# Tiago27Cruz/OctreeRayTracer

Hardware: AMD Instinct MI355X
Metric: Mrays/sec at 3840x2160, 100k spheres, depth 8; 1/2/4/8-GPU scaling (higher is better)
Workload: dtype f32; 1 GPU; c3: 3840x2160 camera rays (spp=1, bounces=1), 100000 spheres, octree depth 8, maxSpheresPerNode 0; width=3840, height=2160, spheres=100000, octree_depth=8, max_spheres_per_node=0, num_samples=1, max_bounces=1, nodes=10953681, indices=5472144, layout=compact, partition=full frame, frames_in_flight=2, rays=traced rays (octree traversals), all bounces and ranks

## Files before the change

octreeraytracer_amd/csrc/host_emulation.inc:

```

namespace {

struct HostScene {
    enum Check {
        kValidate = 1,
        kNoOctree = 2,
        kValidateTree = 4,
        kOrdered = 8,
    };
    ort::KScene S;
    int mode = 2;
    ort::CompactLayout cl;
    std::vector<float> fplanes, fplanes_b;
    std::vector<uint8_t> lut;
    std::vector<uint4> leaf16;
    std::vector<uint2> cam_node;
    const uint8_t* rank_lut = nullptr;
    std::string error;
    HostScene() { std::memset(&S, 0, sizeof(S)); }
    HostScene(const HostScene&) = delete;
    HostScene& operator=(const HostScene&) = delete;

    int build(const float* cr, const float* ma, const float* fr, int32_t n_spheres, const float* node_min, const float* node_max,
              const int32_t* co, const int32_t* oo, const int32_t* cnt, int32_t n_nodes, const int32_t* idx, int64_t n_indices,
// ... 12 lines not shown
            fr2_.resize((size_t)n_spheres * 2);
            for (int32_t i = 0; i < n_spheres; ++i) {
                fr2_[2 * (size_t)i] = fr[4 * (size_t)i];
                fr2_[2 * (size_t)i + 1] = fr[4 * (size_t)i + 1];
            }
            S.sph_ma = (const float4*)ma;
            S.sph_fr = (const float2*)fr2_.data();
        }
        S.n_spheres = n_spheres;
        S.n_nodes = n_nodes;
        lut.resize(kRankLutBytes);
        for (size_t i = 0; i < lut.size(); ++i) lut[i] = ort::rank_lut_entry((uint32_t)i >> 8, (uint32_t)i & 255u);
        if (!tree) return ORT_OK;
        if (layout == ORT_LAYOUT_COMPACT) {
            if (!ort::buildCompactLayout(in, ORT_COMPACT_MAX_DEPTH, cl, error)) return ORT_ERR_UNSUPPORTED;
            if ((checks & kOrdered) && !cl.ordered) return error = "unordered tree", ORT_ERR_UNSUPPORTED;
            mode = 0;
            S.node = (const uint2*)cl.node.data();
            S.kid = (const uint2*)cl.kid.data();
            S.tail_base = (uint32_t)in.n_indices;
            S.leaf_sph = (const float4*)cl.leaf_sph.data();
            S.leaf_idx = cl.leaf_idx.data();
            S.planes = cl.planes.data();
            S.depth = cl.depth;
            if (ort::Masks64::kLeafInline && cl.depth <= 8) {
                fill_leaf16((const uint2*)cl.node.data(), (int64_t)(cl.node.size() / 2), (const uint4*)cl.leaf_sph.data(),
                            (int64_t)(cl.leaf_sph.size() / 4), leaf16);
                S.leaf16 = leaf16.data();
                S.leaf16_bytes = (uint32_t)(16 * leaf16.size());
                if (ort::Masks64::kLeafDedup) {
                    fill_cam_node((const uint2*)cl.node.data(), leaf16, cam_node);
                    S.cam_node = cam_node.data();
                    S.cam_bytes = (uint32_t)(8 * cam_node.size());
                }
            }
            fplanes.resize(ort::fast_plane_floats(cl.depth));
            ort::fill_fast_planes(cl.planes.data(), fplanes.data(), cl.depth);
            fplanes_b.resize(ort::fast_plane_floats(cl.depth, true));
            ort::fill_fast_planes(cl.planes.data(), fplanes_b.data(), cl.depth, true);
            if (cl.ordered) rank_lut = lut.data();
            return ORT_OK;
        }
        mode = 1;
        a_.resize(4 * (size_t)n_nodes);
        b_.resize(4 * (size_t)n_nodes);
        for (int32_t i = 0; i < n_nodes; ++i) {
            for (int k = 0; k < 3; ++k) {
                a_[4 * (size_t)i + k] = node_min[3 * (size_t)i + k];
                b_[4 * (size_t)i + k] = node_max[3 * (size_t)i + k];
            }
            std::memcpy(&a_[4 * (size_t)i + 3], &co[i], 4);
            std::memcpy(&b_[4 * (size_t)i + 3], &oo[i], 4);
        }
        S.nodeA = (const float4*)a_.data();
        S.nodeB = (const float4*)b_.data();
        S.count = cnt;
        S.indices = idx;
        return ORT_OK;
    }

    static void fill_leaf16(const uint2* node, int64_t n, const uint4* leaf_sph, int64_t n_ent, std::vector<uint4>& out) {
        out.resize((size_t)n);
        for (int64_t i = 0; i < n; ++i) {
            const uint2 rec = node[i];
            uint4 sp = make_uint4(0u, 0u, 0u, ort::kLeaf16ListTag);
            if (rec.y == 1u && (int64_t)rec.x < n_ent) sp = leaf_sph[rec.x];
            out[(size_t)i] = ort::leaf16_record(rec, sp);
        }
    }

    static void fill_cam_node(const uint2* node, const std::vector<uint4>& leaf16, std::vector<uint2>& out) {
        const int64_t n = (int64_t)leaf16.size();
        out.resize((size_t)n);
        for (int64_t i = 0; i < n; ++i) {
            const uint2 rec = node[i];
            const uint32_t ab = ort::cam_has_masks(rec, n) ? ort::leaf_repeat_masks(&leaf16[rec.x], rec.y & 0xffu) : 0u;
            out[(size_t)i] = ort::cam_record(rec, ab);
        }
    }

private:
    std::vector<float> zeros_, fr2_, a_, b_;
};

}

extern "C" {

int ort_debug_trace_rays(const float* cr, int32_t n_spheres, const float* node_min, const float* node_max,
                         const int32_t* co, const int32_t* oo, const int32_t* cnt, int32_t n_nodes, const int32_t* idx,
                         int64_t n_indices, const float* rays, int32_t n_rays, int32_t bounce, int32_t* out) {
    try {
        HostScene hs;
        if (int rc = hs.build(cr, nullptr, nullptr, n_spheres, node_min, node_max, co, oo, cnt, n_nodes, idx, n_indices,
                              ORT_LAYOUT_COMPACT, 1, HostScene::kValidate | HostScene::kOrdered))
            return fail(nullptr, rc, hs.error);
        const ort::KScene& S = hs.S;
        const std::vector<float>&fplanes = hs.fplanes, &fplanes_b = hs.fplanes_b;
        const std::vector<uint8_t>& lut = hs.lut;
        ort::LocalFrames lf;
        for (int32_t i = 0; i < n_rays; ++i) {
            ort::Ray r;
            r.o = ort::mk(rays[6 * (size_t)i], rays[6 * (size_t)i + 1], rays[6 * (size_t)i + 2]);
            r.d = ort::mk(rays[6 * (size_t)i + 3], rays[6 * (size_t)i + 4], rays[6 * (size_t)i + 5]);
            ort::Counters cc;
            for (int k = 0; k < 6; ++k) cc.v[k] = 0;
            float tf = 0.0f, tx = 0.0f;
            int ef = -1, ex = -1;
            ort::V3 inv = ort::mk(1.0f / r.d.x, 1.0f / r.d.y, 1.0f / r.d.z);
            const bool fast = ort::fast_prepare(S, r, inv);
            if (fast) {
                if (!bounce) ort::traverse_fast<false>(S, fplanes.data(), lut.data(), r, inv, 0.001f, ORT_MAXFLOAT, ef, tf, lf, cc);
                else if (S.depth <= 8)
                    ort::traverse_fast_t<false, ort::Masks64Plain>(S, fplanes.data(), lut.data(), r, inv, 0.001f, ORT_MAXFLOAT,
                                                                 ef, tf, lf, cc);
                else
                    ort::traverse_fast_t<false, ort::Masks96Lean>(S, fplanes_b.data(), lut.data(), r, inv, 0.001f,
                                                                ORT_MAXFLOAT, ef, tf, lf, cc);
            }
            ort::traverse_compact<false>(S, fplanes.data(), r, 0.001f, ORT_MAXFLOAT, ex, tx, lf, cc);
            int32_t* o = out + 5 * (size_t)i;
            o[0] = fast ? 1 : 0;
            o[1] = ef;
            o[2] = (int32_t)ort::f2u(tf);
            o[3] = ex;
            o[4] = (int32_t)ort::f2u(tx);
        }
        return ORT_OK;
    } catch (const std::exception& ex) {
        return fail(nullptr, ORT_ERR_INTERNAL, ex.what());
    }
}

int ort_debug_split_rays(const float* cr, int32_t n_spheres, const float* node_min, const float* node_max,
                         const int32_t* co, const int32_t* oo, const int32_t* cnt, int32_t n_nodes, const int32_t* idx,
                         int64_t n_indices, const float* rays, int32_t n_rays, int32_t level, int32_t lanes, int32_t* out) {
    try {
        if (lanes < 1 || level < 1) return fail(nullptr, ORT_ERR_INVALID_ARG, "ort_debug_split_rays: lanes, level >= 1");
        HostScene hs;
        if (int rc = hs.build(cr, nullptr, nullptr, n_spheres, node_min, node_max, co, oo, cnt, n_nodes, idx, n_indices,
                              ORT_LAYOUT_COMPACT, 1, HostScene::kValidate | HostScene::kOrdered))
            return fail(nullptr, rc, hs.error);
        const ort::KScene& S = hs.S;
        const std::vector<float>& fplanes = hs.fplanes;
        const std::vector<uint8_t>& lut = hs.lut;
        ort::LocalFrames lf;
        for (int32_t i = 0; i < n_rays; ++i) {
            ort::Ray r;
            r.o = ort::mk(rays[6 * (size_t)i], rays[6 * (size_t)i + 1], rays[6 * (size_t)i + 2]);
            r.d = ort::mk(rays[6 * (size_t)i + 3], rays[6 * (size_t)i + 4], rays[6 * (size_t)i + 5]);
            const ort::V3 inv = ort::mk(1.0f / r.d.x, 1.0f / r.d.y, 1.0f / r.d.z);
            int32_t* o = out + 4 * (size_t)i;
            o[0] = -1;
            o[1] = 0;
            o[2] = 0x7fffffff;
            o[3] = 0;
            if (!ort::fast_path_ok(r, inv, 0.001f, ORT_MAXFLOAT)) continue;
            int best = 0x7fffffff, be = -1, top = 0, owns = 0;
            float bt = 0.0f;
            for (int j = 0; j < lanes; ++j) {
                int pos = 0x7fffffff, e = -1, st = 0, own = 0;
                float t = 0.0f;
                if (S.depth > 8)
                    ort::traverse_split<ort::Masks96Split>(S, fplanes.data(), lut.data(), r, inv, level, lanes, j, pos, e, t, lf, st, own);
                else
                    ort::traverse_split<ort::Masks64Split>(S, fplanes.data(), lut.data(), r, inv, level, lanes, j, pos, e, t, lf, st, own);
// ... 435 lines not shown
    try {
        if (!name || !bytes) return fail(nullptr, ORT_ERR_INVALID_ARG, "ort_debug_layout: null argument");
        HostScene hs;
        if (int rc = hs.build(cr, nullptr, nullptr, n_spheres, node_min, node_max, co, oo, cnt, n_nodes, idx, n_indices,
                              ORT_LAYOUT_COMPACT, 1, HostScene::kValidate))
            return fail(nullptr, rc, hs.error);
        const std::string what = name;
        const int32_t depth = hs.cl.depth, ordered = hs.cl.ordered ? 1 : 0;
        const void* src = nullptr;
        size_t n = 0;
        if (what == "node") src = hs.cl.node.data(), n = 4 * hs.cl.node.size();
        else if (what == "kid") src = hs.cl.kid.data(), n = 4 * hs.cl.kid.size();
        else if (what == "leaf_sph") src = hs.cl.leaf_sph.data(), n = 4 * hs.cl.leaf_sph.size();
        else if (what == "leaf_idx") src = hs.cl.leaf_idx.data(), n = 4 * hs.cl.leaf_idx.size();
        else if (what == "planes") src = hs.cl.planes.data(), n = 4 * hs.cl.planes.size();
        else if (what == "leaf16") src = hs.leaf16.data(), n = 16 * hs.leaf16.size();
        else if (what == "cam_node") src = hs.cam_node.data(), n = 8 * hs.cam_node.size();
        else if (what == "depth") src = &depth, n = 4;
        else if (what == "ordered") src = &ordered, n = 4;
        else return fail(nullptr, ORT_ERR_INVALID_ARG, "ort_debug_layout: unknown array " + what);
        *bytes = (int64_t)n;
        if (!out || n == 0) return ORT_OK;
        if (cap_bytes < (int64_t)n) return fail(nullptr, ORT_ERR_INVALID_ARG, "ort_debug_layout: out too small");
        std::memcpy(out, src, n);
        return ORT_OK;
    } catch (const std::exception& ex) {
        return fail(nullptr, ORT_ERR_INTERNAL, ex.what());
    }
}

int ort_debug_ctx_array(ort_ctx* ctx, const char* name, void* out, int64_t cap_bytes, int64_t* bytes) {
    if (!ctx || !name || !bytes) return fail(ctx, ORT_ERR_INVALID_ARG, "ort_debug_ctx_array: null argument");
    if (!ctx->scene.has_scene) return fail(ctx, ORT_ERR_NO_SCENE, "ort_debug_ctx_array: no scene");
    const std::string what = name;
    const Scene& sc = ctx->scene;
    const int32_t scalars[3] = {sc.depth, sc.ordered ? 1 : 0, sc.layout};
    const char* const scalar_names[3] = {"depth", "ordered", "layout"};
    for (int k = 0; k < 3; ++k)
        if (what == scalar_names[k]) {
            *bytes = 4;
            if (!out) return ORT_OK;
            if (cap_bytes < 4) return fail(ctx, ORT_ERR_INVALID_ARG, "ort_debug_ctx_array: out too small");
            std::memcpy(out, &scalars[k], 4);
            return ORT_OK;
        }
    const DevBuf* b = nullptr;
    if (what == "node") b = &sc.node;
    else if (what == "kid") b = &sc.kid;
    else if (what == "leaf_sph") b = &sc.leaf_sph;
    else if (what == "leaf_idx") b = &sc.leaf_idx;
    else if (what == "planes") b = &sc.planes;
    else if (what == "nk") b = &sc.nk;
    else if (what == "leaf16") b = &sc.leaf16;
    else if (what == "cam_node") b = &sc.cam_node;
    else if (what == "lds_img") b = &sc.lds_img;
    else if (what == "lds_rev") b = &sc.lds_rev;
    else return fail(ctx, ORT_ERR_INVALID_ARG, "ort_debug_ctx_array: unknown array " + what);
    *bytes = b->p ? (int64_t)b->bytes : 0;
    if (!out || *bytes == 0) return ORT_OK;
    if (cap_bytes < *bytes) return fail(ctx, ORT_ERR_INVALID_ARG, "ort_debug_ctx_array: out too small");
    HIPCHK(ctx, hipSetDevice(ctx->device));
    HIPCHK(ctx, hipStreamSynchronize(ctx->stream));
    HIPCHK(ctx, hipMemcpy(out, b->p, b->bytes, hipMemcpyDeviceToHost));
    return ORT_OK;
}

int ort_debug_leaf_forms(uint64_t* out4, int32_t reset) {
    for (int i = 0; i < 4; ++i) {
        if (out4) out4[i] = ort::g_leaf_forms[i];
        if (reset) ort::g_leaf_forms[i] = 0;
    }
    return ORT_OK;
}

int ort_debug_leaf_dedup(uint64_t* out3, int32_t reset) {
    for (int i = 0; i < 2; ++i) {
        if (out3) out3[i] = ort::g_leaf_dedup[i];
        if (reset) ort::g_leaf_dedup[i] = 0;
    }
    if (out3) out3[2] = (uint64_t)ort::Masks64::kLeafDedup;
    return ORT_OK;
}

int ort_debug_pop_coverage(uint64_t* hb_pops, uint64_t* sign_masks, int32_t reset) {
    for (int i = 0; i < 64; ++i)
        if (hb_pops) hb_pops[i] = ort::g_pop_cover[i];
    for (int i = 0; i < 8; ++i)
        if (sign_masks) sign_masks[i] = ort::g_pop_cover[64 + i];
    if (reset)
        for (int i = 0; i < 72; ++i) ort::g_pop_cover[i] = 0;
    return ORT_OK;
}

}
```

octreeraytracer_amd/csrc/ort_internal.h:

```cpp
#pragma once
#include <cstdint>
#include <string>

#include "../../include/ort.h"

namespace ort {
void set_thread_error(const std::string& msg);
const char* thread_error();
}

extern "C" {
int ort_debug_emulate_render(const float* sphere_center_radius, const float* sphere_mat_albedo,
                             const float* sphere_fuzz_ri, int32_t n_spheres, const float* node_min,
                             const float* node_max, const int32_t* children_offset,
                             const int32_t* objects_offset, const int32_t* object_count, int32_t n_nodes,
                             const int32_t* object_indices, int64_t n_indices, int32_t layout,
                             const ort_params* params, const ort_tile* tile, float* rgb_out, uint64_t* counts);
int ort_debug_emulate_render_prefix(const float* sphere_center_radius, const float* sphere_mat_albedo,
                                    const float* sphere_fuzz_ri, int32_t n_spheres, const float* node_min,
                                    const float* node_max, const int32_t* children_offset,
                                    const int32_t* objects_offset, const int32_t* object_count, int32_t n_nodes,
                                    const int32_t* object_indices, int64_t n_indices, int32_t layout,
                                    const ort_params* params, const ort_tile* tile, int32_t samples_done,
                                    float* rgb_out, uint64_t* counts);
// ... 13 lines not shown
                         const float* node_max, const int32_t* children_offset, const int32_t* objects_offset,
                         const int32_t* object_count, int32_t n_nodes, const int32_t* object_indices, int64_t n_indices,
                         const float* rays, int32_t n_rays, int32_t bounce, int32_t* out);
int ort_debug_query_rays(const float* sphere_center_radius, int32_t n_spheres, const float* node_min,
                         const float* node_max, const int32_t* children_offset, const int32_t* objects_offset,
                         const int32_t* object_count, int32_t n_nodes, const int32_t* object_indices, int64_t n_indices,
                         int32_t layout, int32_t use_octree, const float* rays, int64_t n_rays, ort_ray_hit* hits,
                         float* normals);
int ort_debug_query_rays_ex(const float* sphere_center_radius, int32_t n_spheres, const float* node_min,
                            const float* node_max, const int32_t* children_offset, const int32_t* objects_offset,
                            const int32_t* object_count, int32_t n_nodes, const int32_t* object_indices, int64_t n_indices,
                            int32_t layout, int32_t use_octree, const float* rays, int64_t n_rays, int32_t mode,
                            const float* t_range, ort_ray_hit* hits, float* normals);
int ort_debug_camera_query(const float* sphere_center_radius, int32_t n_spheres, const float* node_min,
                           const float* node_max, const int32_t* children_offset, const int32_t* objects_offset,
                           const int32_t* object_count, int32_t n_nodes, const int32_t* object_indices, int64_t n_indices,
                           int32_t layout, const ort_params* params, const ort_tile* tile, int32_t which, float* rays,
                           ort_ray_hit* hits, float* normals);
int ort_debug_radiance_rays(const float* sphere_center_radius, const float* sphere_mat_albedo,
                            const float* sphere_fuzz_ri, int32_t n_spheres, const float* node_min,
                            const float* node_max, const int32_t* children_offset, const int32_t* objects_offset,
                            const int32_t* object_count, int32_t n_nodes, const int32_t* object_indices,
                            int64_t n_indices, int32_t layout, int32_t use_octree, const float* rays,
                            const float* states, int64_t n_rays, int32_t max_depth, int32_t paths, int32_t flags,
                            float* radiance, float* states_out);
int ort_debug_denoise(const ort_denoise_desc* d, const ort_output* output);
int ort_debug_denoise_ex(const ort_denoise_desc_ex* d, const ort_output* output);
int ort_debug_history_update(const ort_params* prev_params, int32_t prev_x0, int32_t prev_y0, const float* prev_a,
                             const float* prev_b, const ort_history_frame* f, float* next_a, float* next_b);
int ort_debug_history_update_ex(const ort_params* prev_params, int32_t prev_x0, int32_t prev_y0, const float* prev_a,
                                const float* prev_b, const ort_history_frame_ex* f, const float* now, const float* snap,
                                int32_t n_spheres, float* next_a, float* next_b);
int ort_debug_history_state(int64_t* st, int32_t op, int32_t n_spheres, int32_t* reads_snapshot);
int ort_debug_gamma(const float* rgb, int64_t n_pixels, float* out);
int ort_debug_emulate_moments(const float* sphere_center_radius, const float* sphere_mat_albedo,
                              const float* sphere_fuzz_ri, int32_t n_spheres, const float* node_min,
                              const float* node_max, const int32_t* children_offset,
                              const int32_t* objects_offset, const int32_t* object_count, int32_t n_nodes,
                              const int32_t* object_indices, int64_t n_indices, int32_t layout,
                              const ort_params* params, const ort_tile* tile, int32_t samples_done,
                              float* mean, float* variance);
int ort_debug_emulate_adaptive(const float* sphere_center_radius, const float* sphere_mat_albedo,
                               const float* sphere_fuzz_ri, int32_t n_spheres, const float* node_min,
                               const float* node_max, const int32_t* children_offset,
                               const int32_t* objects_offset, const int32_t* object_count, int32_t n_nodes,
                               const int32_t* object_indices, int64_t n_indices, int32_t layout,
                               const ort_params* params, const ort_tile* tile, const ort_accum_adaptive* passes,
                               int32_t n_passes, int32_t* counts, float* mean, float* variance);
int ort_debug_adaptive_decision(int32_t k, int32_t n_total, const ort_accum_adaptive* criterion, const float* col, float m2);
int ort_debug_wave_stats(const float* sphere_center_radius, const float* sphere_mat_albedo,
                         const float* sphere_fuzz_ri, int32_t n_spheres, const float* node_min,
                         const float* node_max, const int32_t* children_offset, const int32_t* objects_offset,
                         const int32_t* object_count, int32_t n_nodes, const int32_t* object_indices,
                         int64_t n_indices, const ort_params* params, int32_t block_step, double* stats,
                         int32_t n_stats);
int ort_debug_bounce_walks(const float* sphere_center_radius, const float* sphere_mat_albedo,
                           const float* sphere_fuzz_ri, int32_t n_spheres, const float* node_min, const float* node_max,
                           const int32_t* children_offset, const int32_t* objects_offset, const int32_t* object_count,
                           int32_t n_nodes, const int32_t* object_indices, int64_t n_indices, const ort_params* params,
                           const ort_tile* tile, int32_t bounce, float* rays, int32_t* walks, int64_t cap,
                           int64_t* n_out);
int64_t ort_debug_walk_steps(const float* sphere_center_radius, const float* sphere_mat_albedo,
                             const float* sphere_fuzz_ri, int32_t n_spheres, const float* node_min,
                             const float* node_max, const int32_t* children_offset, const int32_t* objects_offset,
                             const int32_t* object_count, int32_t n_nodes, const int32_t* object_indices,
                             int64_t n_indices, const ort_params* params, int32_t block_step, int32_t* lens,
                             int64_t n_lens, uint16_t* steps, int64_t cap);
int ort_debug_lds_image(int32_t depth, const float* planes, uint32_t* image, int64_t cap_words, int32_t* layout);
int ort_debug_pop_coverage(uint64_t* hb_pops, uint64_t* sign_masks, int32_t reset);
int ort_debug_leaf16(const float* sphere_center_radius, int32_t n_spheres, const float* node_min, const float* node_max,
                     const int32_t* children_offset, const int32_t* objects_offset, const int32_t* object_count,
                     int32_t n_nodes, const int32_t* object_indices, int64_t n_indices, uint32_t* node,
                     uint32_t* leaf_sph, uint32_t* leaf16, int64_t* sizes);
int ort_debug_ctx_leaf16(ort_ctx* ctx, uint32_t* out, int64_t cap, int64_t* n);
int ort_debug_lds_image_rev(int32_t depth, const float* planes, int32_t rev_tables, uint32_t* image, int64_t cap_words,
                            int32_t* layout);
int ort_debug_layout(const float* sphere_center_radius, int32_t n_spheres, const float* node_min, const float* node_max,
                     const int32_t* children_offset, const int32_t* objects_offset, const int32_t* object_count,
                     int32_t n_nodes, const int32_t* object_indices, int64_t n_indices, const char* name, void* out,
                     int64_t cap_bytes, int64_t* bytes);
int ort_debug_ctx_array(ort_ctx* ctx, const char* name, void* out, int64_t cap_bytes, int64_t* bytes);
int ort_debug_leaf_forms(uint64_t* out4, int32_t reset);
int ort_debug_leaf_dedup(uint64_t* out3, int32_t reset);
int64_t ort_debug_walk_steps_ex(const float* sphere_center_radius, const float* sphere_mat_albedo, const float* sphere_fuzz_ri,
                                int32_t n_spheres, const float* node_min, const float* node_max, const int32_t* children_offset,
                                const int32_t* objects_offset, const int32_t* object_count, int32_t n_nodes,
                                const int32_t* object_indices, int64_t n_indices, const ort_params* p, int32_t block_step,
                                int32_t production, int32_t* lens, int64_t n_lens, uint16_t* steps, int64_t cap);
}
```

octreeraytracer_amd/csrc/render_fast_state.inc:

```
namespace ort {
struct Masks64 {
    static constexpr bool kLdsScene = false;
    static constexpr bool kInlineLeaves = true;
    static constexpr bool kRevPlanes = true;
    static constexpr bool kPreMid = true;
    static constexpr bool kKidSkip = false;
    static constexpr bool kPopTable = true;
    static constexpr bool kLeafInline = true;
    static constexpr bool kLeafDedup = true;
    uint64_t m;
    ORT_FN void clear() { m = 0; }
    ORT_FN bool empty() const { return m == 0; }
    ORT_FN void put(int L, uint32_t rev) { m |= (uint64_t)rev << (8 * L); }
    ORT_FN int pop() {
        const int hb = 63 - __builtin_clzll(m);
        m ^= (uint64_t)1 << hb;
        return hb;
    }
    ORT_FN int peek() const { return 63 - __builtin_clzll(m); }
    ORT_FN void drop(uint32_t lo, uint32_t hi) { m ^= ((uint64_t)hi << 32) | lo; }
    ORT_FN bool take(int hb) {
        const uint64_t b = (uint64_t)1 << hb;
        const bool t = (m & b) != 0;
        m &= ~b;
        return t;
    }
    ORT_FN void uniform() {
#if defined(__HIP_DEVICE_COMPILE__)
        m = ((uint64_t)(uint32_t)__builtin_amdgcn_readfirstlane((int)(uint32_t)(m >> 32)) << 32) |
            (uint32_t)__builtin_amdgcn_readfirstlane((int)(uint32_t)m);
#endif
    }
};
struct Masks96 {
    static constexpr bool kLdsScene = false;
    static constexpr bool kInlineLeaves = false;
    static constexpr bool kLeafInline = false;
    static constexpr bool kLeafDedup = false;
    static constexpr bool kPreMid = false;
    static constexpr bool kRevPlanes = false;
    static constexpr bool kPopTable = false;
    static constexpr bool kKidSkip = true;
    static constexpr int kSplit = 2;
    uint64_t lo;
    uint32_t hi;
    ORT_FN void clear() { lo = 0; hi = 0; }
    ORT_FN bool empty() const { return (lo | hi) == 0; }
    ORT_FN void put(int L, uint32_t rev) {
        if (L >= kSplit) lo |= (uint64_t)rev << (8 * (L - kSplit));
        else hi |= rev << (8 * L);
    }
    ORT_FN int pop() {
        if (lo) {
            const int hb = 63 - __builtin_clzll(lo);
            lo ^= (uint64_t)1 << hb;
            return 8 * kSplit + hb;
        }
        const int hb = 31 - __builtin_clz(hi);
        hi ^= 1u << hb;
        return hb;
    }
    ORT_FN bool take(int hb) {
        if (hb >= 8 * kSplit) {
            const uint64_t b = (uint64_t)1 << (hb - 8 * kSplit);
            const bool t = (lo & b) != 0;
            lo &= ~b;
            return t;
        }
        const uint32_t b = 1u << hb;
        const bool t = (hi & b) != 0;
        hi &= ~b;
        return t;
    }    ORT_FN void uniform() {
#if defined(__HIP_DEVICE_COMPILE__)
        lo = ((uint64_t)(uint32_t)__builtin_amdgcn_readfirstlane((int)(uint32_t)(lo >> 32)) << 32) |
             (uint32_t)__builtin_amdgcn_readfirstlane((int)(uint32_t)lo);
        hi = (uint32_t)__builtin_amdgcn_readfirstlane((int)hi);
#endif
    }
};

template <class Masks>
struct FastStateT {
    static_assert(!Masks::kPreMid || (Masks::kRevPlanes && Masks::kInlineLeaves), "mid planes in the pop: never a level-D leaf");
    static_assert(!Masks::kPopTable || (Masks::kRevPlanes && Masks::kInlineLeaves), "the pop table has no level-D entries");
    static_assert(!Masks::kLeafInline || (Masks::kInlineLeaves && !Masks::kKidSkip), "leaf16 records: inline leaf children, no skip");
    static_assert(!Masks::kLeafDedup || Masks::kLeafInline, "repeat masks: the leaf16 records");
    V3 d;
    float ya;
    float oA, oB, oC, iA, iB, iC;
    const float* pl0;
    uint32_t aA, aB, aC;
    uint32_t h4;
#if defined(__HIP_DEVICE_COMPILE__)
    ORT_FN float plane(uint32_t a) const { return *(const __attribute__((address_space(3))) float*)(size_t)a; }
    static ORT_FN uint32_t table_base(const float* planes) {
        return (uint32_t)(size_t)(const __attribute__((address_space(3))) float*)planes;
    }
    ORT_FN uint4 entry(uint32_t a) const { return *(const __attribute__((address_space(3))) uint4*)(size_t)a; }
#else
    ORT_FN float plane(uint32_t off) const { return *(const float*)((const char*)pl0 + off); }
    ORT_FN uint4 entry(uint32_t off) const {
        uint4 e;
        __builtin_memcpy(&e, (const char*)pl0 + off, 16);
        return e;
    }
    static ORT_FN uint32_t table_base(const float*) { return 0u; }
#endif
    const float* pA;
    const float* pB;
    const float* pC;
    int sA, sB, sC;
    float tNA, tFA, tNB, tFB, tNC, tFC;
    float tMA, tMB, tMC;
    uint32_t cP;
    uint32_t otab;
    int node, depth;
    uint2 kd;
    uint2 rec;
    float closest;
    int hitEntry;
    uint32_t kc_id;
    float kc_e;
    Masks masks;
    ORT_FN bool hit() const { return hitEntry >= 0; }
    ORT_FN float pl(const float* p, int s, int idx) const { return *at(p, s, idx); }
    const float* nA;
    const float* nB;
    const float* nC;
    ORT_FN const float* at(const float* p, int s, int idx) const {
        return (const float*)((const char*)p + imul24(s, idx));
    }
    ORT_FN float plA(int idx) const { return pl(pA, sA, idx); }
    ORT_FN float plB(int idx) const { return pl(pB, sB, idx); }
    ORT_FN float plC(int idx) const { return pl(pC, sC, idx); }
    ORT_FN int cA() const { return (int)(cP & 1023u); }
    ORT_FN int cB() const { return (int)((cP >> 10) & 1023u); }
    ORT_FN int cC() const { return (int)(cP >> 20); }
    ORT_FN Ray ray() const {
        const bool swap = (otab >> 1) & 1u;
        Ray r;
        r.o = mk(swap ? oB : oA, swap ? oA : oB, oC);
        r.d = d;
        return r;
    }
};
using FastState = FastStateT<Masks96>;
struct Masks96Lean : Masks96 {
    static constexpr bool kRevPlanes = true;
};
struct Masks64Plain : Masks64 {
    static constexpr bool kInlineLeaves = false;
    static constexpr bool kLeafInline = false;
    static constexpr bool kLeafDedup = false;
    static constexpr bool kPopTable = false;
    static constexpr bool kPreMid = false;
    static constexpr bool kKidSkip = true;
};
struct Masks64PlainLds : Masks64Plain {
    static constexpr bool kLdsScene = true;
};

struct Masks64Split : Masks64Plain {
    static constexpr bool kKidSkip = false;
};
struct Masks96Split : Masks96 {
    static constexpr bool kKidSkip = false;
};
}
```

octreeraytracer_amd/csrc/render_fast_walk.inc:

```
namespace ort {
#if defined(__HIP_DEVICE_COMPILE__)
ORT_FN uint4 lds_u4(uint32_t a) { return *(const __attribute__((address_space(3))) uint4*)(size_t)a; }
#endif
template <bool CAM = false, class Masks>
ORT_FN void fetch_rec(const KScene& S, int i, bool kid, FastStateT<Masks>& st) {
    if constexpr (CAM) {
        static_assert(!Masks::kKidSkip && !Masks::kLdsScene, "cam_node: the depth <= 8 camera walk, no kid entries");
        st.rec = fetch_cam(S, i);
        return;
    }
#if defined(__HIP_DEVICE_COMPILE__)
    if constexpr (Masks::kLdsScene) {
        const uint4 v = lds_u4(S.lds_nk + 16u * (uint32_t)i);
        st.rec = make_uint2(v.x, v.y);
        st.kd = make_uint2(v.z, v.w);
        return;
    }
#endif
    if (Masks::kKidSkip && kid && S.nk) {
        const uint4 v = fetch_nk(S, i);
        st.rec = make_uint2(v.x, v.y);
        st.kd = make_uint2(v.z, v.w);
        return;
    }
    st.rec = fetch_node(S, i);
    if (kid) st.kd = fetch_kid(S, i);
}

template <int CAM = -1, class Masks>
ORT_FN bool fast_begin(const KScene& S, const float* planes, const uint8_t* rank_lut, const Ray& r, V3 inv, float t_min,
                       float t_max, FastStateT<Masks>& st) {
    const int D = S.depth;
    const int top = 1 << D;
    const uint32_t nx = f2u(inv.x) >> 31, ny = f2u(inv.y) >> 31, nz = f2u(inv.z) >> 31;
    const uint32_t m = (nz << 2) | (nx << 1) | ny;
    const bool swap = nx != 0;
    const uint32_t gA = swap ? ny : nx, gB = swap ? nx : ny, gC = nz;
    st.d = r.d;
    st.ya = 1.0f / dot(r.d, r.d);
    st.oA = swap ? r.o.y : r.o.x;
    st.oB = swap ? r.o.x : r.o.y;
    st.oC = r.o.z;
    st.iA = swap ? inv.y : inv.x;
    st.iB = swap ? inv.x : inv.y;
    st.iC = inv.z;
    st.otab = (swap ? 0x75643120u : 0x76543210u) ^ (m * 0x11111111u);
    if (Masks::kRevPlanes) {
        st.pl0 = planes;
        const uint32_t b0 = FastStateT<Masks>::table_base(planes);
        const uint32_t T = (uint32_t)fast_rev_T(D), S3 = 3u * T;
        st.aA = b0 + 4u * ((swap ? S3 : 0u) + (gA ? T : 0u));
        st.aB = b0 + 4u * ((swap ? 0u : S3) + (gB ? T : 0u));
        st.aC = b0 + 4u * (2u * S3 + (gC ? T : 0u));
        st.h4 = 2u * (uint32_t)top;
        const uint32_t t4 = 4u * (uint32_t)top;
        st.tNA = st.iA * (st.plane(st.aA) - st.oA);
        st.tFA = st.iA * (st.plane(st.aA + t4) - st.oA);
        st.tNB = st.iB * (st.plane(st.aB) - st.oB);
        st.tFB = st.iB * (st.plane(st.aB + t4) - st.oB);
        st.tNC = st.iC * (st.plane(st.aC) - st.oC);
        st.tFC = st.iC * (st.plane(st.aC + t4) - st.oC);
        if (Masks::kPreMid) {
            const uint32_t hm = st.h4 & ~3u;
            st.tMA = st.iA * (st.plane(st.aA + hm) - st.oA);
            st.tMB = st.iB * (st.plane(st.aB + hm) - st.oB);
            st.tMC = st.iC * (st.plane(st.aC + hm) - st.oC);
        }
    } else {
        const int S1 = fast_axis_floats(D);
        st.pA = planes + (swap ? S1 : 0) + (gA ? top : 0);
        st.pB = planes + (swap ? 0 : S1) + (gB ? top : 0);
        st.pC = planes + 2 * S1 + (gC ? top : 0);
        st.sA = gA ? -4 : 4;
        st.sB = gB ? -4 : 4;
        st.sC = gC ? -4 : 4;
        st.tNA = st.iA * (st.plA(0) - st.oA);
        st.tFA = st.iA * (st.plA(top) - st.oA);
        st.tNB = st.iB * (st.plB(0) - st.oB);
        st.tFB = st.iB * (st.plB(top) - st.oB);
        st.tNC = st.iC * (st.plC(0) - st.oC);
        st.tFC = st.iC * (st.plC(top) - st.oC);
        st.cP = 0;
        st.nA = st.pA;
        st.nB = st.pB;
        st.nC = st.pC;
    }
    st.node = 0;
    fetch_rec<(CAM < 0 ? Masks::kLeafDedup : CAM != 0)>(S, 0, Masks::kKidSkip && S.kid, st);
    st.depth = 0;
    st.closest = t_max;
    st.hitEntry = -1;
    st.kc_id = ~0u;
    st.kc_e = 0.0f;
    st.masks.clear();
    return fmin3(st.tFA, st.tFB, st.tFC) >= fmax3(st.tNA, st.tNB, st.tNC);
}

#if ORT_ANALYSIS
inline unsigned long long g_leaf_forms[4];
inline unsigned long long g_leaf_dedup[2];
inline bool g_leaf_list_call = false;
#endif

template <bool COUNT, class Masks>
ORT_FN bool leaf_tests(const KScene& S, FastStateT<Masks>& st, int off, int n, float ntmin, Counters& cnt) {
    const Ray r = st.ray();
    const float a = dot(r.d, r.d);
    for (int i = 0; i < n; ++i) {
#if defined(__HIP_DEVICE_COMPILE__)
        float4 sp;
        if constexpr (Masks::kLdsScene) {
            const uint4 v = lds_u4(S.lds_sph + 16u * (uint32_t)(off + i));
            sp = make_float4(__uint_as_float(v.x), __uint_as_float(v.y), __uint_as_float(v.z), __uint_as_float(v.w));
        } else {
            sp = fetch_sphere(S, off + i);
        }
#else
        const float4 sp = fetch_sphere(S, off + i);
#endif
        if (COUNT) cnt.v[2] += 1;
        float t;
        const bool h = sphere_hit_fast(r, a, st.ya, sp, ntmin, st.closest, t);
#if ORT_ANALYSIS && !defined(__HIP_DEVICE_COMPILE__)
        if (g_leaf_list_call) {
            g_leaf_forms[2] += 1;
            g_leaf_forms[3] += h ? 1 : 0;
        }
#endif
        if (h) {
            st.closest = t;
            st.hitEntry = off + i;
            if (COUNT) cnt.v[3] += 1;
        }
    }
    if (!COUNT && Masks::kKidSkip) {
        const bool rej = n == 1 && !st.hit();
        st.kc_id = rej ? (uint32_t)off - S.tail_base : st.kc_id;
        st.kc_e = rej ? ntmin : st.kc_e;
    }
    return st.hit();
}

ORT_FN uint32_t child_drops(float tNA, float tNB, float tMA, float tMB, float tFA, float tFB, float nN, float nF,
                            float cN, float cF) {
    uint32_t drop = 0;
#if defined(__HIP_DEVICE_COMPILE__)
    float e, x;
#define ORT_C(EA, EB, EC, XA, XB, XC)                                                         \
    "v_max3_f32 %[e], " EA ", " EB ", " EC "\n\tv_min3_f32 %[x], " XA ", " XB ", " XC "\n\t" \
    "v_sub_f32 %[x], %[x], %[e]\n\tv_alignbit_b32 %[d], %[d], %[x], 31\n\t"
    asm("v_mov_b32 %[d], 0\n\t"
        ORT_C("%[NA]", "%[NB]", "%[nN]", "%[MA]", "%[MB]", "%[cN]")
        ORT_C("%[NA]", "%[MB]", "%[nN]", "%[MA]", "%[FB]", "%[cN]")
        ORT_C("%[MA]", "%[NB]", "%[nN]", "%[FA]", "%[MB]", "%[cN]")
        ORT_C("%[MA]", "%[MB]", "%[nN]", "%[FA]", "%[FB]", "%[cN]")
        ORT_C("%[NA]", "%[NB]", "%[nF]", "%[MA]", "%[MB]", "%[cF]")
        ORT_C("%[NA]", "%[MB]", "%[nF]", "%[MA]", "%[FB]", "%[cF]")
        ORT_C("%[MA]", "%[NB]", "%[nF]", "%[FA]", "%[MB]", "%[cF]")
        ORT_C("%[MA]", "%[MB]", "%[nF]", "%[FA]", "%[FB]", "%[cF]")
        : [d] "=&v"(drop), [e] "=&v"(e), [x] "=&v"(x)
        : [NA] "v"(tNA), [NB] "v"(tNB), [MA] "v"(tMA), [MB] "v"(tMB), [FA] "v"(tFA), [FB] "v"(tFB), [nN] "v"(nN),
          [nF] "v"(nF), [cN] "v"(cN), [cF] "v"(cF));
#undef ORT_C
#else
#define ORT_CHILD(EA, EB, EC, XA, XB, XC) drop = (drop << 1) | (f2u(fmin3(XA, XB, XC) - fmax3(EA, EB, EC)) >> 31);
    ORT_CHILD(tNA, tNB, nN, tMA, tMB, cN)
    ORT_CHILD(tNA, tMB, nN, tMA, tFB, cN)
    ORT_CHILD(tMA, tNB, nN, tFA, tMB, cN)
    ORT_CHILD(tMA, tMB, nN, tFA, tFB, cN)
    ORT_CHILD(tNA, tNB, nF, tMA, tMB, cF)
    ORT_CHILD(tNA, tMB, nF, tMA, tFB, cF)
    ORT_CHILD(tMA, tNB, nF, tFA, tMB, cF)
    ORT_CHILD(tMA, tMB, nF, tFA, tFB, cF)
#undef ORT_CHILD
#endif
    return drop;
}

template <class Masks>
ORT_FN bool leaf16_tests(const KScene& S, FastStateT<Masks>& st, int kid, uint4 lr, float ntmin, Counters& cnt) {
    if (!(lr.w >> 31)) {
        const Ray r = st.ray();
        const float a = dot(r.d, r.d);
        float t;
        const bool h = sphere_hit_fast(r, a, st.ya, make_float4(u2f(lr.x), u2f(lr.y), u2f(lr.z), u2f(lr.w)), ntmin,
                                       st.closest, t);
#if ORT_ANALYSIS && !defined(__HIP_DEVICE_COMPILE__)
        g_leaf_forms[0] += 1;
        g_leaf_forms[1] += h ? 1 : 0;
#endif
        if (h) {
            st.closest = t;
            st.hitEntry = kid | kLeafIdFlag;
        }
        return st.hit();
    }
#if ORT_ANALYSIS && !defined(__HIP_DEVICE_COMPILE__)
    g_leaf_list_call = true;
    const bool hl = leaf_tests<false>(S, st, (int)lr.x, (int)lr.y, ntmin, cnt);
    g_leaf_list_call = false;
    return hl;
#else
    return leaf_tests<false>(S, st, (int)lr.x, (int)lr.y, ntmin, cnt);
#endif
}

template <bool COUNT, class Masks>
ORT_FN bool leaf_kids(const KScene& S, FastStateT<Masks>& st, int co, uint32_t keep, float tNA, float tMA, float tNB,
                      float tMB, float nN, float nF, uint32_t rep, Counters& cnt) {
    uint32_t todo = keep;
    while (todo) {
        const int hb = 31 - __builtin_clz(todo);
        todo ^= 1u << hb;
#if ORT_ANALYSIS && !defined(__HIP_DEVICE_COMPILE__)
        int dropped = 0;
#endif
        if constexpr (!COUNT && Masks::kLeafDedup) {
#if defined(__HIP_DEVICE_COMPILE__)
            uint32_t a;
            asm("v_bfe_i32 %[a], %[rep], %[hb], 1\n\tv_and_b32 %[a], %[a], %[rep]\n\t"
                "v_bfi_b32 %[t], %[a], 0, %[t]"
                : [a] "=&v"(a), [t] "+v"(todo)
                : [rep] "v"(rep), [hb] "v"(hb));
#else
            const uint32_t cut = ((rep >> hb) & 1u) ? rep : 0u;
#if ORT_ANALYSIS
            dropped = __builtin_popcount(todo & cut);
#endif
            todo &= ~cut;
#endif
        }
#if ORT_ANALYSIS && !defined(__HIP_DEVICE_COMPILE__)
        if (!COUNT && Masks::kLeafInline) g_leaf_dedup[0] += 1;
#endif
        const uint32_t R = 7u - (uint32_t)hb;
        const int kid = co + (int)((st.otab >> (4 * R)) & 15u);
        constexpr bool kRec16 = !COUNT && Masks::kLeafInline;
        uint4 lr = make_uint4(0u, 0u, 0u, 0u);
        if constexpr (kRec16) {
            lr = fetch_leaf16(S, kid);
        } else {
            const uint2 lrec = fetch_node(S, kid);
            lr.x = lrec.x;
            lr.y = lrec.y;
        }
        if (COUNT) cnt.v[0] += 1;
#if defined(__HIP_DEVICE_COMPILE__)
        float eA, eB, eC;
        {
            uint32_t m;
            asm("v_bfe_i32 %[m], %[R], 1, 1\n\tv_bfi_b32 %[a], %[m], %[MA], %[NA]\n\t"
                "v_bfe_i32 %[m], %[R], 0, 1\n\tv_bfi_b32 %[b], %[m], %[MB], %[NB]\n\t"
                "v_bfe_i32 %[m], %[R], 2, 1\n\tv_bfi_b32 %[c], %[m], %[CF], %[CN]"
                : [a] "=&v"(eA), [b] "=&v"(eB), [c] "=&v"(eC), [m] "=&v"(m)
                : [R] "v"(R), [MA] "v"(tMA), [NA] "v"(tNA), [MB] "v"(tMB), [NB] "v"(tNB), [CF] "v"(nF), [CN] "v"(nN));
        }
#else
        const float eA = (R & 2u) ? tMA : tNA, eB = (R & 1u) ? tMB : tNB, eC = (R & 4u) ? nF : nN;
#endif
        const float ntmin = fmax3(eA, eB, eC);
        bool h;
        if constexpr (kRec16) h = leaf16_tests(S, st, kid, lr, ntmin, cnt);
        else h = leaf_tests<COUNT>(S, st, (int)lr.x, (int)lr.y, ntmin, cnt);
#if ORT_ANALYSIS && !defined(__HIP_DEVICE_COMPILE__)
        g_leaf_dedup[1] += h ? 0ull : (unsigned long long)dropped;
#endif
        todo = h ? 0u : todo;
    }
    return st.hit();
}

template <bool COUNT, class Masks, class Frames>
ORT_FN bool fast_visit(const KScene& S, const uint8_t* rank_lut, FastStateT<Masks>& st, Frames& fr, Counters& cnt) {
    const int D = S.depth;
    const uint2 rec = st.rec;
    if (COUNT) cnt.v[0] += 1;
    if (rec.y & ORT_INTERNAL_FLAG) {
        const int co = (int)rec.x;
        if (COUNT) {
            const long long rem = (long long)S.n_nodes - (long long)co;
            cnt.v[1] += (unsigned long long)(rem >= 8 ? 8 : (rem > 0 ? rem : 0));
        }
        uint32_t cm = rec.y & 0xffu;
        if (!COUNT && Masks::kKidSkip && S.kid) {
            const uint2 kd = st.kd;
            const uint32_t m = (((kd.x & 0xffffffu) == st.kc_id) ? (kd.x >> 24) : 0u) |
                               (((kd.y & 0xffffffu) == st.kc_id) ? (kd.y >> 24) : 0u);
            const float ptmin = fmax_tmin(fmax3(st.tNA, st.tNB, st.tNC));
            cm &= ~(m & (0u - (uint32_t)(st.kc_e <= ptmin)));
        }
        const uint32_t rcm = rank_lut[((st.otab & 7u) << 8) | cm];
        const int h = 1 << (D - 1 - st.depth);
        float tMA, tMB, tMC;
        if (Masks::kPreMid) {
            tMA = st.tMA;
            tMB = st.tMB;
            tMC = st.tMC;
        } else if (Masks::kRevPlanes) {
            const uint32_t h4 = st.h4;
            tMA = st.iA * (st.plane(st.aA + h4) - st.oA);
            tMB = st.iB * (st.plane(st.aB + h4) - st.oB);
            tMC = st.iC * (st.plane(st.aC + h4) - st.oC);
        } else {
            tMA = st.iA * (*st.at(st.nA, st.sA, h) - st.oA);
            tMB = st.iB * (*st.at(st.nB, st.sB, h) - st.oB);
            tMC = st.iC * (*st.at(st.nC, st.sC, h) - st.oC);
        }
        const float tNA = st.tNA, tNB = st.tNB, tNC = st.tNC, tFA = st.tFA, tFB = st.tFB, tFC = st.tFC;
        const float nN = fmax_tmin(tNC), nF = fmax_tmin(tMC);
        const float cN = fmin2(tMC, st.closest), cF = fmin2(tFC, st.closest);
        const uint32_t keep = rcm & ~child_drops(tNA, tNB, tMA, tMB, tFA, tFB, nN, nF, cN, cF) & 0xffu;
        if (Masks::kInlineLeaves && (rec.y & ORT_LEAFKIDS_FLAG)) {
            uint32_t rep = 0;
            if constexpr (!COUNT && Masks::kLeafDedup) {
                rep = rank_lut[((st.otab & 7u) << 8) | ((rec.y >> 8) & 0xffu)];
            }
            if (leaf_kids<COUNT>(S, st, co, keep, tNA, tMA, tNB, tMB, nN, nF, rep, cnt)) return true;
        } else {
            st.masks.put(st.depth, keep);
            fr.setCo(st.depth, co);
        }
    } else {
        const float ntmin = st.depth == 0 ? kFastTMin : fmax_tmin(fmax3(st.tNA, st.tNB, st.tNC));
        if (leaf_tests<COUNT>(S, st, (int)rec.x, (int)rec.y, ntmin, cnt)) return true;
    }
    return false;
}

#if ORT_ANALYSIS
inline unsigned long long g_pop_cover[72];
#endif

template <bool COUNT, class Masks, class Frames>
ORT_FN void fast_pop(const KScene& S, FastStateT<Masks>& st, Frames& fr);

template <bool COUNT, class Masks, class Frames>
ORT_FN bool fast_step(const KScene& S, const uint8_t* rank_lut, FastStateT<Masks>& st, Frames& fr, Counters& cnt) {
    if (fast_visit<COUNT>(S, rank_lut, st, fr, cnt)) return true;
    if (st.masks.empty()) return true;
    fast_pop<COUNT>(S, st, fr);
    return false;
}

template <bool COUNT, class Masks, class Frames>
ORT_FN void fast_pop(const KScene& S, FastStateT<Masks>& st, Frames& fr) {
    const int D = S.depth;
    int hb;
    if constexpr (Masks::kPopTable) hb = st.masks.peek();
    else hb = st.masks.pop();
    const int L = hb >> 3;
    const uint32_t rk = (uint32_t)(~hb) & 7u;
    const int w = 1 << (D - 1 - L);
    st.depth = L + 1;
    st.node = fr.getCo(L) + (int)((st.otab >> (4 * rk)) & 15u);
    fetch_rec<(!COUNT && Masks::kLeafDedup)>(S, st.node, !COUNT && Masks::kKidSkip && S.kid, st);
#if ORT_ANALYSIS && !defined(__HIP_DEVICE_COMPILE__)
    if (Masks::kInlineLeaves && Masks::kRevPlanes) {
        g_pop_cover[hb & 63] += 1;
        g_pop_cover[64 + (st.otab & 7u)] += 1;
    }
#endif
    if (Masks::kRevPlanes) {
        uint32_t w4;
        if constexpr (Masks::kPopTable) {
            const uint32_t ta = FastStateT<Masks>::table_base(st.pl0) + (uint32_t)kPopTableOff + 16u * (uint32_t)hb;
            const uint4 e = st.entry(ta);
            st.aA = (st.aA & e.x) | e.y;
            st.aB = (st.aB & e.x) | e.z;
            st.aC = (st.aC & e.x) | e.w;
            const uint4 e2 = st.entry(ta + (uint32_t)kPopTable2);
            w4 = e2.x;
            st.h4 = e2.y;
            st.masks.drop(e2.z, e2.w);
        } else {
            w4 = 4u << (D - 1 - L);
            st.h4 = w4 >> 1;
            const uint32_t m8 = ~(2u * w4 - 1u);
            const uint32_t s = (uint32_t)(D + 1 - L);
            st.aA = (st.aA & m8) | (((rk >> 1) & 1u) << s);
            st.aB = (st.aB & m8) | ((rk & 1u) << s);
            st.aC = (st.aC & m8) | (((rk >> 2) & 1u) << s);
        }
        st.tNA = st.iA * (st.plane(st.aA) - st.oA);
        st.tFA = st.iA * (st.plane(st.aA + w4) - st.oA);
        st.tNB = st.iB * (st.plane(st.aB) - st.oB);
        st.tFB = st.iB * (st.plane(st.aB + w4) - st.oB);
        st.tNC = st.iC * (st.plane(st.aC) - st.oC);
        st.tFC = st.iC * (st.plane(st.aC + w4) - st.oC);
        if (Masks::kPreMid) {
            st.tMA = st.iA * (st.plane(st.aA + st.h4) - st.oA);
            st.tMB = st.iB * (st.plane(st.aB + st.h4) - st.oB);
            st.tMC = st.iC * (st.plane(st.aC + st.h4) - st.oC);
        }
    } else {
// ... 88 lines not shown
```

octreeraytracer_amd/csrc/render_lds_image.inc:

```
namespace ort {
ORT_FN bool fast_rev_planes(int depth) { return depth <= 8; }
ORT_FN int fast_rev_T(int depth) { return depth <= 8 ? 256 : 1 << depth; }
ORT_FN int fast_axis_floats(int depth, bool rev) { return rev ? 3 * fast_rev_T(depth) : (1 << depth) + 1; }
ORT_FN int fast_axis_floats(int depth) { return fast_axis_floats(depth, fast_rev_planes(depth)); }
ORT_FN int fast_plane_floats(int depth, bool rev) {
    return rev ? 7 * fast_rev_T(depth) + (1 << depth) + 1 : 3 * fast_axis_floats(depth, false);
}
ORT_FN int fast_plane_floats(int depth) { return fast_plane_floats(depth, fast_rev_planes(depth)); }
constexpr int kPopEntries = 56;
constexpr int kPopTableOff = 12 * 256 - 16 * kPopEntries;
constexpr int kPopTable2 = 12 * 256;
static_assert(kPopTableOff % 16 == 0 && kPopTableOff >= 4 * (2 * 256 + 1), "the pop table overlaps the reversed table");
ORT_FN bool fast_pop_table(int depth, bool rev) { return rev && depth <= 8; }
ORT_FN uint32_t pop_table_word(int depth, int table, int hb, int k) {
    const int L = hb >> 3;
    if (hb >= 8 * (depth - 1)) return 0u;
    const uint32_t rk = (uint32_t)(~hb) & 7u;
    const uint32_t s = (uint32_t)(depth + 1 - L);
    const uint32_t w4 = 1u << s;
    if (table == 0) {
        if (k == 0) return ~(2u * w4 - 1u);
        const uint32_t bit = k == 1 ? (rk >> 1) & 1u : (k == 2 ? rk & 1u : (rk >> 2) & 1u);
        return bit << s;
    }
    if (k == 0) return w4;
    if (k == 1) return w4 >> 1;
    return (uint32_t)(((uint64_t)1 << hb) >> (k == 2 ? 0 : 32));
}
struct LdsLayout {
    int lut;
    int frames;
    int pop;
};
ORT_FN LdsLayout lds_layout(int depth, bool rev) {
    const int pb = (4 * fast_plane_floats(depth, rev) + 15) & ~15;
    const int T = fast_rev_T(depth);
    LdsLayout l;
    l.pop = fast_pop_table(depth, rev) ? kPopTableOff : -1;
    if (rev && 4 * (2 * T - (1 << depth) - 1) >= 2048) {
        l.lut = 12 * T - 2048;
        l.frames = pb;
    } else {
        l.lut = pb;
        l.frames = pb + 2048;
    }
    return l;
}
ORT_FN void fill_fast_planes(const float* fwd, float* out, int depth, bool rev, int i0 = 0, int step = 1) {
    const int P1 = (1 << depth) + 1;
    const int S = fast_axis_floats(depth, rev);
    const int T = fast_rev_T(depth);
    const int n = fast_plane_floats(depth, rev);
    const bool pop = fast_pop_table(depth, rev);
    for (int o = i0; o < n; o += step) {
        const int a = o / S, r = o - a * S;
        uint32_t u = 0u;
        if (r < P1) u = f2u(fwd[a * P1 + r]);
        else if (rev && r >= T && r - T < P1) u = f2u(fwd[a * P1 + (P1 - 1 - (r - T))]);
        else if (pop && a < 2 && 4 * r >= kPopTableOff) {
            const int i = r - kPopTableOff / 4;
            u = pop_table_word(depth, a, i >> 2, i & 3);
        }
        __builtin_memcpy(out + o, &u, 4);
    }
}
ORT_FN void fill_fast_planes(const float* fwd, float* out, int depth) {
    fill_fast_planes(fwd, out, depth, fast_rev_planes(depth));
}
}
```

Before: 6228 Mrays/s.

## Replace child_drops with sign-bit comparison index into precomputed order tables

In the octree child-visit step, the per-child drop mask is now computed from twelve sign bits of time-comparison differences. These bits index two 64-entry constant tables that are ANDed to give the keep mask, replacing the previous child_drops arithmetic. The device version is hand-written inline assembly using v_sub/v_alignbit. At the camera root, fast_begin also clears the child mask when the ray interval is empty. The change aims to shorten the per-node ALU sequence, at the cost of scalar or constant memory lookups, and it depends on the tables matching child_drops exactly, for which debug and validation entry points are added.

```diff
diff --git a/octreeraytracer_amd/csrc/host_emulation.inc b/octreeraytracer_amd/csrc/host_emulation.inc
--- a/octreeraytracer_amd/csrc/host_emulation.inc
+++ b/octreeraytracer_amd/csrc/host_emulation.inc
@@ -118,6 +118,10 @@
 private:
     std::vector<float> zeros_, fr2_, a_, b_;
 };
+
+__global__ void k_order_tables(uint8_t* out) {
+    if (threadIdx.x < sizeof(ort::OrderTables)) out[threadIdx.x] = ort::g_order_tables.b[threadIdx.x];
+}
 
 }
 
@@ -719,6 +723,77 @@
     return ORT_OK;
 }
 
+int ort_debug_child_order(int32_t mode, const float* in, int64_t n, const float* tmins, int32_t n_tmin,
+                          const float* closests, int32_t n_closest, uint64_t* out) {
+    if (!out) return fail(nullptr, ORT_ERR_INVALID_ARG, "ort_debug_child_order: no output");
+    if (mode == 2) {
+        for (int i = 0; i < 5; ++i) {
+            out[i] = ort::g_order_visits[i];
+            if (n) ort::g_order_visits[i] = 0;
+        }
+        out[5] = (uint64_t)ort::Masks64::kOrderBits;
+        return ORT_OK;
+    }
+    if (mode == 3) {
+        for (int i = 0; i < 128; ++i) out[i] = ort::kOrderTablesHost.b[i];
+        return ORT_OK;
+    }
+    if (mode == 4) {
+        uint8_t* d = nullptr;
+        uint8_t t[sizeof(ort::OrderTables)];
+        if (hipMalloc((void**)&d, sizeof(t)) != hipSuccess) return fail(nullptr, ORT_ERR_INTERNAL, "ort_debug_child_order: hipMalloc failed");
+        hipLaunchKernelGGL(k_order_tables, dim3(1), dim3(128), 0, 0, d);
+        hipError_t e = hipGetLastError();
+        if (e == hipSuccess) e = hipMemcpy(t, d, sizeof(t), hipMemcpyDeviceToHost);
+        (void)hipFree(d);
+        if (e != hipSuccess) return fail(nullptr, ORT_ERR_INTERNAL, "ort_debug_child_order: reading the tables failed");
+        for (int i = 0; i < 128; ++i) out[i] = t[i];
+        return ORT_OK;
+    }
+    if ((mode != 0 && mode != 1) || !in || n < 0) return fail(nullptr, ORT_ERR_INVALID_ARG, "ort_debug_child_order: bad args");
+    auto both = [&](const float* v, uint32_t& a, uint32_t& b) {
+        a = ~ort::child_drops(v[0], v[1], v[2], v[3], v[4], v[5], v[6], v[7], v[8], v[9]) & 0xffu;
+        b = ort::child_order_keep(v[0], v[1], v[2], v[3], v[4], v[5], v[6], v[7], v[8], v[9]);
+    };
+    if (mode == 0) {
+        for (int64_t i = 0; i < n; ++i) {
+            uint32_t a, b;
+            both(in + 10 * i, a, b);
+            out[2 * i] = a;
+            out[2 * i + 1] = b;
+        }
+        return ORT_OK;
+    }
+    if (!tmins || !closests || n_tmin < 1 || n_closest < 1) return fail(nullptr, ORT_ERR_INVALID_ARG, "ort_debug_child_order: bad args");
+    for (int64_t i = 1; i < n; ++i)
+        if (!(in[i - 1] <= in[i])) return fail(nullptr, ORT_ERR_INVALID_ARG, "ort_debug_child_order: grid not ascending");
+    struct Tri { float v[3]; float operator[](int i) const { return v[i]; } };
+    std::vector<Tri> tri;
+    for (int64_t i = 0; i < n; ++i)
+        for (int64_t j = i; j < n; ++j)
+            for (int64_t k = j; k < n; ++k) tri.push_back(Tri{{in[i], in[j], in[k]}});
+    for (int i = 0; i < 4; ++i) out[i] = 0;
+    for (const auto& A : tri)
+        for (const auto& B : tri)
+            for (const auto& Cx : tri)
+                for (int32_t ti = 0; ti < n_tmin; ++ti)
+                    for (int32_t ci = 0; ci < n_closest; ++ci) {
+                        const float v[10] = {A[0], B[0], A[1], B[1], A[2], B[2], fmaxf(Cx[0], tmins[ti]), fmaxf(Cx[1], tmins[ti]),
+                                             fminf(Cx[1], closests[ci]), fminf(Cx[2], closests[ci])};
+                        uint32_t a, b;
+                        both(v, a, b);
+                        const bool premise = ort::fmin3(v[4], v[5], v[9]) >= ort::fmax3(v[0], v[1], v[6]);
+                        if (premise) {
+                            out[0] += 1;
+                            out[1] += a != b;
+                        } else {
+                            out[2] += 1;
+                            out[3] += a != 0;
+                        }
+                    }
+    return ORT_OK;
+}
+
 int ort_debug_pop_coverage(uint64_t* hb_pops, uint64_t* sign_masks, int32_t reset) {
     for (int i = 0; i < 64; ++i)
         if (hb_pops) hb_pops[i] = ort::g_pop_cover[i];
diff --git a/octreeraytracer_amd/csrc/ort_internal.h b/octreeraytracer_amd/csrc/ort_internal.h
--- a/octreeraytracer_amd/csrc/ort_internal.h
+++ b/octreeraytracer_amd/csrc/ort_internal.h
@@ -119,6 +119,8 @@
 int ort_debug_ctx_array(ort_ctx* ctx, const char* name, void* out, int64_t cap_bytes, int64_t* bytes);
 int ort_debug_leaf_forms(uint64_t* out4, int32_t reset);
 int ort_debug_leaf_dedup(uint64_t* out3, int32_t reset);
+int ort_debug_child_order(int32_t mode, const float* in, int64_t n, const float* tmins, int32_t n_tmin,
+                          const float* closests, int32_t n_closest, uint64_t* out);
 int64_t ort_debug_walk_steps_ex(const float* sphere_center_radius, const float* sphere_mat_albedo, const float* sphere_fuzz_ri,
                                 int32_t n_spheres, const float* node_min, const float* node_max, const int32_t* children_offset,
                                 const int32_t* objects_offset, const int32_t* object_count, int32_t n_nodes,
diff --git a/octreeraytracer_amd/csrc/render_fast_state.inc b/octreeraytracer_amd/csrc/render_fast_state.inc
--- a/octreeraytracer_amd/csrc/render_fast_state.inc
+++ b/octreeraytracer_amd/csrc/render_fast_state.inc
@@ -8,6 +8,7 @@
     static constexpr bool kPopTable = true;
     static constexpr bool kLeafInline = true;
     static constexpr bool kLeafDedup = true;
+    static constexpr bool kOrderBits = true;
     uint64_t m;
     ORT_FN void clear() { m = 0; }
     ORT_FN bool empty() const { return m == 0; }
@@ -40,6 +41,7 @@
     static constexpr bool kPreMid = false;
     static constexpr bool kRevPlanes = false;
     static constexpr bool kPopTable = false;
+    static constexpr bool kOrderBits = false;
     static constexpr bool kKidSkip = true;
     static constexpr int kSplit = 2;
     uint64_t lo;
@@ -86,6 +88,7 @@
     static_assert(!Masks::kPopTable || (Masks::kRevPlanes && Masks::kInlineLeaves), "the pop table has no level-D entries");
     static_assert(!Masks::kLeafInline || (Masks::kInlineLeaves && !Masks::kKidSkip), "leaf16 records: inline leaf children, no skip");
     static_assert(!Masks::kLeafDedup || Masks::kLeafInline, "repeat masks: the leaf16 records");
+    static_assert(!Masks::kOrderBits || Masks::kLeafDedup, "order bits: the depth <= 8 camera walk (fast_begin's CAM)");
     V3 d;
     float ya;
     float oA, oB, oC, iA, iB, iC;
@@ -155,6 +158,7 @@
     static constexpr bool kLeafDedup = false;
     static constexpr bool kPopTable = false;
     static constexpr bool kPreMid = false;
+    static constexpr bool kOrderBits = false;
     static constexpr bool kKidSkip = true;
 };
 struct Masks64PlainLds : Masks64Plain {
diff --git a/octreeraytracer_amd/csrc/render_fast_walk.inc b/octreeraytracer_amd/csrc/render_fast_walk.inc
--- a/octreeraytracer_amd/csrc/render_fast_walk.inc
+++ b/octreeraytracer_amd/csrc/render_fast_walk.inc
@@ -26,6 +26,10 @@
     st.rec = fetch_node(S, i);
     if (kid) st.kd = fetch_kid(S, i);
 }
+
+#if ORT_ANALYSIS
+inline unsigned long long g_order_visits[5];
+#endif
 
 template <int CAM = -1, class Masks>
 ORT_FN bool fast_begin(const KScene& S, const float* planes, const uint8_t* rank_lut, const Ray& r, V3 inv, float t_min,
@@ -93,6 +97,13 @@
     st.kc_id = ~0u;
     st.kc_e = 0.0f;
     st.masks.clear();
+    if constexpr (Masks::kOrderBits && (CAM < 0 ? Masks::kLeafDedup : CAM != 0)) {
+        const float E = fmax3(st.tNA, st.tNB, fmax_tmin(st.tNC)), X = fmin3(st.tFA, st.tFB, fmin2(st.tFC, t_max));
+#if ORT_ANALYSIS && !defined(__HIP_DEVICE_COMPILE__)
+        g_order_visits[4] += (st.rec.y & ORT_INTERNAL_FLAG) && !(X >= E);
+#endif
+        if ((st.rec.y & ORT_INTERNAL_FLAG) && !(X >= E)) st.rec.y &= ~0xffu;
+    }
     return fmin3(st.tFA, st.tFB, st.tFC) >= fmax3(st.tNA, st.tNB, st.tNC);
 }
 
@@ -177,6 +188,61 @@
     return drop;
 }
 
+ORT_FN void child_order_index(float tNA, float tNB, float tMA, float tMB, float tFA, float tFB, float nN, float nF,
+                              float cN, float cF, uint32_t& i1, uint32_t& i2) {
+    const float E = fmax3(tNA, tNB, nN), X = fmin3(tFA, tFB, cF);
+    uint32_t a = 0, b = 0;
+#define ORT_BIT(I, P, Q) I = (I << 1) | (f2u((P) - (Q)) >> 31);
+    ORT_BIT(a, tMA, E)
+    ORT_BIT(a, tMB, E)
+    ORT_BIT(a, cN, E)
+    ORT_BIT(a, X, tMA)
+    ORT_BIT(a, X, tMB)
+    ORT_BIT(a, X, nF)
+    ORT_BIT(b, tMA, tMB)
+    ORT_BIT(b, tMB, tMA)
+    ORT_BIT(b, tMA, nF)
+    ORT_BIT(b, cN, tMA)
+    ORT_BIT(b, tMB, nF)
+    ORT_BIT(b, cN, tMB)
+#undef ORT_BIT
+    i1 = a;
+    i2 = b;
+}
+ORT_FN uint32_t child_order_keep(float tNA, float tNB, float tMA, float tMB, float tFA, float tFB, float nN, float nF,
+                                 float cN, float cF) {
+#if defined(__HIP_DEVICE_COMPILE__)
+    uint32_t a1, a2;
+    float e;
+#define ORT_B0(I, T, P, Q) "v_sub_f32 " T ", " P ", " Q "\n\tv_lshrrev_b32 " I ", 31, " T "\n\t"
+#define ORT_B(I, T, P, Q) "v_sub_f32 " T ", " P ", " Q "\n\tv_alignbit_b32 " I ", " I ", " T ", 31\n\t"
+    asm("v_max3_f32 %[e], %[NA], %[NB], %[nN]\n\t"
+        ORT_B0("%[a1]", "%[a2]", "%[MA]", "%[e]")
+        ORT_B("%[a1]", "%[a2]", "%[MB]", "%[e]")
+        ORT_B("%[a1]", "%[a2]", "%[cN]", "%[e]")
+        "v_min3_f32 %[a2], %[FA], %[FB], %[cF]\n\t"
+        ORT_B("%[a1]", "%[e]", "%[a2]", "%[MA]")
+        ORT_B("%[a1]", "%[e]", "%[a2]", "%[MB]")
+        ORT_B("%[a1]", "%[e]", "%[a2]", "%[nF]")
+        ORT_B0("%[a2]", "%[e]", "%[MA]", "%[MB]")
+        ORT_B("%[a2]", "%[e]", "%[MB]", "%[MA]")
+        ORT_B("%[a2]", "%[e]", "%[MA]", "%[nF]")
+        ORT_B("%[a2]", "%[e]", "%[cN]", "%[MA]")
+        ORT_B("%[a2]", "%[e]", "%[MB]", "%[nF]")
+        ORT_B("%[a2]", "%[e]", "%[cN]", "%[MB]")
+        : [a1] "=&v"(a1), [a2] "=&v"(a2), [e] "=&v"(e)
+        : [NA] "v"(tNA), [NB] "v"(tNB), [MA] "v"(tMA), [MB] "v"(tMB), [FA] "v"(tFA), [FB] "v"(tFB), [nN] "v"(nN),
+          [nF] "v"(nF), [cN] "v"(cN), [cF] "v"(cF));
+#undef ORT_B0
+#undef ORT_B
+    return (uint32_t)g_order_tables.b[a1] & (uint32_t)g_order_tables.b[(size_t)a2 + 64];
+#else
+    uint32_t i1, i2;
+    child_order_index(tNA, tNB, tMA, tMB, tFA, tFB, nN, nF, cN, cF, i1, i2);
+    return (uint32_t)kOrderTablesHost.b[i1] & (uint32_t)kOrderTablesHost.b[64u + i2];
+#endif
+}
+
 template <class Masks>
 ORT_FN bool leaf16_tests(const KScene& S, FastStateT<Masks>& st, int kid, uint4 lr, float ntmin, Counters& cnt) {
     if (!(lr.w >> 31)) {
@@ -309,7 +375,19 @@
         const float tNA = st.tNA, tNB = st.tNB, tNC = st.tNC, tFA = st.tFA, tFB = st.tFB, tFC = st.tFC;
         const float nN = fmax_tmin(tNC), nF = fmax_tmin(tMC);
         const float cN = fmin2(tMC, st.closest), cF = fmin2(tFC, st.closest);
-        const uint32_t keep = rcm & ~child_drops(tNA, tNB, tMA, tMB, tFA, tFB, nN, nF, cN, cF) & 0xffu;
+        uint32_t keep;
+        if constexpr (!COUNT && Masks::kOrderBits) {
+#if ORT_ANALYSIS && !defined(__HIP_DEVICE_COMPILE__)
+            g_order_visits[0] += 1;
+            g_order_visits[1] += !(tNA <= tMA && tMA <= tFA && tNB <= tMB && tMB <= tFB && nN <= nF && cN <= cF);
+            g_order_visits[2] += st.depth > 0 && !(fmin3(tFA, tFB, cF) >= fmax3(tNA, tNB, nN));
+            g_order_visits[3] += (rcm & child_order_keep(tNA, tNB, tMA, tMB, tFA, tFB, nN, nF, cN, cF)) !=
+                                 (rcm & ~child_drops(tNA, tNB, tMA, tMB, tFA, tFB, nN, nF, cN, cF) & 0xffu);
+#endif
+            keep = rcm & child_order_keep(tNA, tNB, tMA, tMB, tFA, tFB, nN, nF, cN, cF);
+        } else {
+            keep = rcm & ~child_drops(tNA, tNB, tMA, tMB, tFA, tFB, nN, nF, cN, cF) & 0xffu;
+        }
         if (Masks::kInlineLeaves && (rec.y & ORT_LEAFKIDS_FLAG)) {
             uint32_t rep = 0;
             if constexpr (!COUNT && Masks::kLeafDedup) {
diff --git a/octreeraytracer_amd/csrc/render_lds_image.inc b/octreeraytracer_amd/csrc/render_lds_image.inc
--- a/octreeraytracer_amd/csrc/render_lds_image.inc
+++ b/octreeraytracer_amd/csrc/render_lds_image.inc
@@ -27,6 +27,32 @@
     if (k == 1) return w4 >> 1;
     return (uint32_t)(((uint64_t)1 << hb) >> (k == 2 ? 0 : 32));
 }
+constexpr uint32_t order_kill_set(int cond) {
+    const uint32_t far = (uint32_t)(0x142421412000ull >> (4 * cond)) & 7u;
+    const uint32_t near = (uint32_t)(0x414212000412ull >> (4 * cond)) & 7u;
+    uint32_t kill = 0;
+    for (uint32_t R = 0; R < 8; ++R)
+        if ((R & far) == far && (R & near) == 0) kill |= 0x80u >> R;
+    return kill;
+}
+constexpr uint32_t order_table_entry(int table, int index) {
+    uint32_t keep = 0xffu;
+    for (int j = 0; j < 6; ++j)
+        if ((index >> (5 - j)) & 1) keep &= ~order_kill_set(6 * table + j);
+    return keep;
+}
+struct OrderTables {
+    uint8_t b[128];
+};
+constexpr OrderTables make_order_tables() {
+    OrderTables t{};
+    for (int i = 0; i < 128; ++i) t.b[i] = (uint8_t)order_table_entry(i >> 6, i & 63);
+    return t;
+}
+#if defined(__HIPCC__)
+static __device__ const OrderTables g_order_tables = make_order_tables();
+#endif
+static constexpr OrderTables kOrderTablesHost = make_order_tables();
 struct LdsLayout {
     int lut;
     int frames;
```

After: 6503 Mrays/s, median of 6. 4.4% higher.
